# zrudnick/bramble

Hardware: AMD Instinct MI355X
Metric: projected alignments/sec vs GENCODE-scale annotation (higher is better)
Workload: dtype u32; 1 GPU; device-resident (inputs already in HBM, packed rows left in HBM): 10M paired-end 2x100 short reads (name-collated, unstranded) vs GENCODE-shaped synthetic annotation (250836 transcripts, 1684128 transcript-exon rows, 25 refs); BASELINE.json configs[1]; group_lanes=8, seed=0xb4a3b1e

## Files before the change

bramble_amd/csrc/direct_kernels.inc:

```

#define WAVE_SYNC()                                                \
  do {                                                             \
    __builtin_amdgcn_fence(__ATOMIC_RELEASE, "workgroup");         \
    __builtin_amdgcn_wave_barrier();                               \
    __builtin_amdgcn_fence(__ATOMIC_ACQUIRE, "workgroup");         \
  } while (0)

__global__ void __launch_bounds__(256) k_name_seed(DirectArgs D) {
  const int64_t g = (int64_t)blockIdx.x * blockDim.x + threadIdx.x;
  if (g >= D.n_groups) return;
  const uint32_t a0 = D.group_off[g];
  const uint32_t no = D.name_off[a0];
  Mt64Lazy gen;
  gen.seed(hash_bytes(D.names + no, D.name_off[a0 + 1] - no));
  D.rnd0[g] = gen();
}
__device__ __forceinline__ uint32_t pick_from(uint64_t z0, const uint8_t *name, uint64_t len, uint32_t n) {
  uint64_t hi, lo;
  mul64wide(z0, (uint64_t)n, hi, lo);
  if (lo < (uint64_t)n) {
    const uint64_t thr = (0 - (uint64_t)n) % (uint64_t)n;
    if (lo < thr) return primary_pick(name, len, n);
  }
  return (uint32_t)hi;
// ... 164 lines not shown
  __shared__ uint16_t sh_mops[EM ? 256 : 1];
  const int lane = threadIdx.x;
  if (EM) {
    for (int t = lane; t < 256; t += 64) sh_mops[t] = (uint16_t)((merge_action(t >> 4, t & 15u) << 8) | merge_ops(t >> 4, t & 15u));
    WAVE_SYNC();
  }
  const DevIndex &ix = A.ix;
  const DevCfg &cfg = A.cfg;
  const uint32_t n_work = *D.n_big;
  for (uint32_t w = blockIdx.x; w < n_work; w += gridDim.x) {
    if (D.side_used[1]) {
      if (EM) return;
      unsigned long long need = 0;
      for (uint64_t v = (uint64_t)w + (uint64_t)lane * gridDim.x; v < n_work; v += 64ull * gridDim.x) need += side_need(D.n_matches[D.big_list[v]]);
#pragma unroll
      for (int d = 32; d >= 1; d >>= 1) need += __shfl_down(need, d, 64);
      if (lane == 0 && need) atomicAdd(D.side_used, need);
      return;
    }
    const uint32_t a = D.big_list[w];
    const uint32_t nm = D.n_matches[a];
    if (EM && D.n_kept[a] == 0) continue;
    const uint4 hd = A.head[a], hd2 = A.head2[a], rg = A.ranges[a];
    const uint32_t n_seg = hd.z, rid = hd.w >> 2;
    if (n_seg == 0 || nm == 0) continue;
    const uint2 q0 = make_uint2(hd.x, hd.y);
    const int st0 = (n_seg == 1) ? ST_ONLY : ST_FIRST;
    const uint32_t sb[2] = {ix.slab_off[2 * rid], ix.slab_off[2 * rid + 1]}, se[2] = {ix.slab_off[2 * rid + 1], ix.slab_off[2 * rid + 2]};
    const uint32_t n0 = rg.y - rg.x, n_items = n0 + (rg.w - rg.z);
    unsigned long long off = 0;
    uint4 E = make_uint4(0, 0, 0, 0);
    if (!EM) {
      const unsigned long long need = side_need(nm);
      if (lane == 0) off = atomicAdd(D.side_used, need);
      off = ((unsigned long long)__shfl((uint32_t)(off >> 32), 0) << 32) | __shfl((uint32_t)off, 0);
      if (off + need > D.side_cap) { if (lane == 0) D.side_used[1] = 1; continue; }
      if (lane == 0) D.fm[a] = make_uint2((uint32_t)off, (uint32_t)(off >> 32));
    } else {
      const uint2 f = D.fm[a];
      off = (unsigned long long)f.x | ((unsigned long long)f.y << 32);
      { const uint2 gd = D.gd[a], dp = D.dpos[a]; E = make_uint4(gd.x, gd.y, dp.x, dp.y); }
    }
    const uint32_t c0 = A.cigar_off[a];
    ReadCtx rd;
    rd.n_seg = n_seg; rd.seg = A.seg + (size_t)c0 + (size_t)a; rd.real = A.cigar + c0; rd.n_real = A.cigar_off[a + 1] - c0; rd.q12 = hd2;
    uint32_t seen = 0;
    for (uint32_t base = 0; base < n_items; base += 64) {
// ... 359 lines not shown
  }
  sh_v[wv][lane] = v;
#pragma unroll
  for (int c = 0; c < 2; c++) {
    const uint32_t mine = (nk && fast == (c == 0)) ? nk : 0u;
    const uint64_t have = __ballot(mine != 0u);
    if (!have) continue;
    uint32_t inc = mine;
#pragma unroll
    for (int d = 1; d < 64; d <<= 1) { const uint32_t up = __shfl_up(inc, d); if (lane >= d) inc += up; }
    const uint32_t total = __shfl(inc, 63), first = __shfl(pos, (int)__builtin_ctzll(have));
    __builtin_amdgcn_wave_barrier();
    sh_pre[wv][lane] = inc - mine;
    WAVE_SYNC();
    for (uint32_t e = lane; e < total; e += 64) {
      int l = 0;
#pragma unroll
      for (int st = 32; st; st >>= 1) if (sh_pre[wv][l + st] <= e) l += st;
      D.m_aln[first + e] = sh_v[wv][l];
    }
  }
}

template <int CLS>
__global__ void __launch_bounds__(256, CLS == 1 ? 8 : 6) k_emit_rows(ProjectArgs A, DirectArgs D, int64_t first, int64_t n_end) {
  __shared__ uint32_t sh_cig[CLS == 1 ? 1 : 256 * LDS_SLOT];
  __shared__ uint16_t sh_mops[CLS == 1 ? 1 : 256];
  if (CLS != 1) {
    sh_mops[threadIdx.x] = (uint16_t)((merge_action(threadIdx.x >> 4, threadIdx.x & 15u) << 8) | merge_ops(threadIdx.x >> 4, threadIdx.x & 15u));
    __syncthreads();
  }
  const int64_t e64 = first + (int64_t)blockIdx.x * blockDim.x + threadIdx.x;
  if (e64 >= n_end) return;
  const DevIndex &ix = A.ix;
  const DevCfg &cfg = A.cfg;
  typedef uint32_t ntl4 __attribute__((ext_vector_type(4)));
  typedef uint32_t ntl2 __attribute__((ext_vector_type(2)));
  const uint32_t a = __builtin_nontemporal_load(D.m_aln + e64);
  if (a == 0xffffffffu) return;
  const ntl4 hd_ = __builtin_nontemporal_load((const ntl4 *)(A.head + a)), rg_ = __builtin_nontemporal_load((const ntl4 *)(A.ranges + a));
  const ntl2 f_ = __builtin_nontemporal_load((const ntl2 *)(D.fm + a)), gd_ = __builtin_nontemporal_load((const ntl2 *)(D.gd + a)), dp_ = __builtin_nontemporal_load((const ntl2 *)(D.dpos + a));
  const uint4 hd = make_uint4(hd_.x, hd_.y, hd_.z, hd_.w), rg = make_uint4(rg_.x, rg_.y, rg_.z, rg_.w);
  const uint2 f = make_uint2(f_.x, f_.y), gd = make_uint2(gd_.x, gd_.y), dp = make_uint2(dp_.x, dp_.y);
  const uint4 E = make_uint4(gd.x, gd.y, dp.x, dp.y);
  const uint32_t is_fast = CLS == 1;
  uint4 hd2 = make_uint4(0, 0, 0, 0);
  uint32_t c0 = 0, c1 = 0;
  RealCig rc;
  if (CLS != 1) { hd2 = A.head2[a]; c0 = A.cigar_off[a]; c1 = A.cigar_off[a + 1]; }
  else if (hd.z == 2) hd2 = A.head2[a];
  const uint32_t n_seg = hd.z, rid = hd.w >> 2;
  const uint2 q0 = make_uint2(hd.x, hd.y);
  const int st0 = (n_seg == 1) ? ST_ONLY : ST_FIRST;
  const uint32_t n0 = rg.y - rg.x;
  if (CLS != 1) rc.fetch(A.cigar + c0, c1 - c0);
  const uint32_t k = (uint32_t)e64 - E.w;
  const uint64_t fmask = (uint64_t)f.x | ((uint64_t)f.y << 32);
  uint64_t mm = fmask;
  for (uint32_t j = 0; j < k; j++) mm &= mm - 1;
  const uint32_t item = (uint32_t)(__ffsll((long long)mm) - 1);
  const int s = item < n0 ? 0 : 1;
  const uint32_t row = s == 0 ? rg.x + item : rg.z + (item - n0);
  const uint4 r_a = ix.s_row[2 * (size_t)row], r_b = ix.s_row[2 * (size_t)row + 1];
  const uint32_t gs = r_a.x, gend = r_a.y;
  const uint4 pay = make_uint4(r_b.x, r_b.y, r_a.w, r_b.z);
  uint32_t c = 0;
  {
    for (uint64_t m2 = fmask; m2;) {
      uint32_t t8[8]; bool ok[8];
#pragma unroll
      for (int u = 0; u < 8; u++) {
        ok[u] = m2 != 0;
        const uint32_t b = ok[u] ? (uint32_t)(__ffsll((long long)m2) - 1) : item;
        m2 &= m2 - 1;
        t8[u] = ix.s_tid[b < n0 ? rg.x + b : rg.z + (b - n0)];
      }
#pragma unroll
      for (int u = 0; u < 8; u++) c += (ok[u] && t8[u] < pay.x) ? 1u : 0u;
    }
  }
  Hit h0;
  classify(s == 1, st0, q0.x, q0.y, gs, gend, pay.z, cfg, h0);
  if (is_fast) {
    const uint32_t os = q0.x > gs ? q0.x : gs, oe = q0.y < gend ? q0.y : gend;
    uint32_t ml = oe - os, pos = h0.pos, r_ins = h0.right_ins, junc_in = 0;
    bool r_exact = h0.right_ins == 0 && h0.right_gap == 0;
    if (n_seg == 2) {
      const uint2 q1 = make_uint2(hd2.x, hd2.y);
      const uint4 e1 = next_row(make_uint4(gs, gend, pay.z, 0), make_uint2(r_a.z, r_b.w), s == 1);
      Hit hh;
      classify(s == 1, ST_LAST, q1.x, q1.y, e1.x, e1.y, e1.z, cfg, hh);
      ml += (q1.y < e1.y ? q1.y : e1.y) - q1.x;
      pos = s == 0 ? h0.pos : hh.pos;
      r_ins = hh.right_ins; r_exact = hh.right_ins == 0 && hh.right_gap == 0;
      junc_in = 2;
    }
    uint32_t w0, w1 = 0, w2 = 0, n_out;
    if (h0.left_ins) { w0 = CIG_GEN(h0.left_ins, OP_S); w1 = CIG_GEN(ml, OP_M); n_out = 2; if (r_ins) { w2 = CIG_GEN(r_ins, OP_S); n_out = 3; } }
    else { w0 = CIG_GEN(ml, OP_M); n_out = 1; if (r_ins) { w1 = CIG_GEN(r_ins, OP_S); n_out = 2; } }
    const uint32_t junc = junc_in + ((h0.left_ins == 0 && h0.left_gap == 0) ? 1u : 0u) + (r_exact ? 1u : 0u);
    uint64_t cref = (uint64_t)w0 | ((uint64_t)w1 << 32);
    if (n_out == 3) {
      cref = D.cig_base[a] + (uint64_t)c * (n_seg == 2 ? 3u + 2u * 10u : 1u + 2u * 6u);
      uint32_t *slot = A.cig_arena + cref;
      slot[0] = w0; slot[1] = w1; slot[2] = w2;
    }
    write_row(D, E, a, c, pay.x, pos, n_out, s == 1, cref, junc, ml);
    return;
  }
  if (CLS == 1) return;
  ReadCtx rd;
  rd.n_seg = n_seg; rd.seg = A.seg + (size_t)c0 + (size_t)a; rd.real = A.cigar + c0; rd.n_real = c1 - c0; rd.q12 = hd2;
  const uint4 *Ex = ix.tx_ex + pay.w;
  const uint32_t i0 = pay.y & 0x7fffffffu;
  CandOut p1;
  bool plain = false;
  const uint32_t sb = ix.slab_off[2 * rid + s], se = ix.slab_off[2 * rid + s + 1];
  if (n_seg == 1) { p1.alive = true; p1.fwpos = h0.pos; p1.rcpos = h0.pos; p1.n_seg = 1; p1.n_gex = 1; p1.i_lastm = i0; p1.last_right_ins = h0.right_ins; p1.last_right_gap = h0.right_gap; }
  else if (!cfg.long_reads && !cfg.ignore_small_exons) {
    plain = true;
    p1.alive = true; p1.fwpos = h0.pos; p1.rcpos = h0.pos; p1.n_seg = n_seg; p1.n_gex = n_seg; p1.i_lastm = i0;
    p1.last_right_ins = 0; p1.last_right_gap = 0;
  }
  else p1 = walk_pass1(ix, cfg, rd, Ex, s == 1, sb, se, i0, make_uint4(gs, gend, pay.z, 0), make_uint2(r_a.z, r_b.w), q0, h0);
  const uint32_t ideal_cap = 4u * n_seg + 2u;
  const uint32_t cap = rd.n_real + 2u * ideal_cap;
// ... 57 lines not shown
```

bramble_amd/csrc/kernels.h:

```cpp
#pragma once
#include <hip/hip_runtime.h>
#include <stdint.h>

#include "device_types.h"
#include "ksw_types.h"

namespace br {

enum {
  TOT_MATCHES = 0,
  TOT_ARENA = 1,
  TOT_SIMPLE = 2,
  TOT_ROWS = 3,
  TOT_RAW = 4,
  TOT_RESCUE_PROB = 5,
  TOT_RESCUE_SEQ = 6,
  TOT_WIDE_CIGAR = 7,
  TOT_SMALL_CNT = 8,
  TOT_PARSE_CIGAR = 12,
  TOT_PARSE_NAMES = 13,
  TOT_PARSE_GROUPS = 14,
  TOT_PARSE_SEQ = 15,
  TOT_BAM_LONG = 16,
  TOT_BAM_BYTES = 17,
// ... 355 lines not shown
};
struct SoaArgs {
  int64_t n;
  const uint64_t *cigar_off64, *name_off64, *seq_off64;
  uint32_t *cigar_off, *name_off, *seq_off;
  const uint8_t *names;
  const uint32_t *cigar;
  uint32_t *isnew;
  uint32_t *maxima;
};
void launch_soa_fields(hipStream_t st, const SoaArgs &S);
void launch_rec_fields(hipStream_t st, const ParseArgs &P);
void launch_group_off(hipStream_t st, const ParseArgs &P);
void launch_rec_copy(hipStream_t st, const ParseArgs &P);
void launch_mates(hipStream_t st, const ParseArgs &P);
void launch_seq_src(hipStream_t st, const ParseArgs &P);
void launch_seq_ascii(hipStream_t st, const ParseArgs &P);
void launch_bam_size(hipStream_t st, const BamArgs &B);
void launch_bam_encode(hipStream_t st, const BamArgs &B, int lanes);

struct SegExtra {
  const uint32_t *group_off; uint32_t *aln_group; int64_t n_groups;
  uint64_t *zero_a; int n_zero_a; uint64_t *zero_b; int n_zero_b;
};
void launch_segment(hipStream_t st, int64_t n_aln, const int32_t *ref_id, const int32_t *ref_start,
                    const uint16_t *flags, const int8_t *xs, const int8_t *ts, const uint32_t *cigar_off,
                    const uint32_t *cigar, const DevCfg &cfg, uint32_t n_refs, uint2 *seg, AlnMeta *meta,
                    uint4 *head, uint4 *head2, uint32_t *fast_flag, const SegExtra *extra = nullptr);
void launch_project(hipStream_t st, const ProjectArgs &A, bool emit, int group_lanes, int n_blocks);
void launch_count(hipStream_t st, const CountArgs &C, int group_lanes, int n_blocks, int part);
void launch_project_fa(hipStream_t st, const ProjectArgs &A, const FaArgs &F, int mode, int n_blocks);
void launch_fa_fill(hipStream_t st, const ProjectArgs &A, const FaArgs &F, int64_t n_prob);
void launch_ksw(hipStream_t st, const KswArgs &K, int n_blocks);
void launch_ksw_bin(hipStream_t st, const KswFastArgs &A);
void launch_ksw_dp(hipStream_t st, const KswFastArgs &A, int bin);
void launch_ksw_trace(hipStream_t st, const KswFastArgs &A, int bin);
uint32_t ksw_dp_resident_groups(int bin, int n_cu);
size_t ksw_prob_bytes();
size_t ksw_res_bytes();
void launch_expand(hipStream_t st, const ProjectArgs &A);
void launch_emit_dense(hipStream_t st, const ProjectArgs &A, int64_t n_matches, int64_t n_simple, int part);
void launch_emit_dense_fa(hipStream_t st, const ProjectArgs &A, const FaArgs &F, int64_t n_matches);
int64_t scan_tiles_for(int64_t n);
void launch_scan(hipStream_t st, const ScanArgs &S, int mode, void *out, bool out64, uint64_t *total_out);
void launch_group_ids(hipStream_t st, int64_t n_groups, const uint32_t *group_off, uint32_t *aln_group);
bool launch_scan3(hipStream_t st, ScanArgs S, uint32_t *match_off, uint64_t *cig_base, uint32_t *fast_pre,
                  uint64_t *total_out3, const ProjectArgs *expand = nullptr);
// ... 11 lines not shown
```

bramble_amd/csrc/pipeline.cpp:

```cpp
#include <algorithm>
#include <cstring>
#include <vector>

#include "ctx.h"

int ensure_side_stream(br_ctx *c) {
  if (c->side_stream) return BR_OK;
  HIPCHK(hipStreamCreateWithPriority(&c->side_stream, hipStreamNonBlocking, 0));
  for (auto &p : c->side_ev) for (auto &e : p) HIPCHK(hipEventCreateWithFlags(&e, hipEventDisableTiming));
  return BR_OK;
}

int run_ksw(br_ctx *c, hipStream_t st, const KswRun &R) {
  if (R.n_prob <= 0) return BR_OK;
  const uint64_t n_all = (uint64_t)R.n_prob;
  const uint64_t qmax = std::max<uint64_t>(R.qmax, 1), tmax = std::max<uint64_t>(R.tmax, 1);
  KswArgs K{};
  K.n_prob = R.n_prob; K.probs = R.probs; K.results = R.results; K.seq_arena = R.seq_arena; K.clip_ops = R.clip_ops;
  K.stats = R.stats;
  K.raw_out = R.raw_out; K.raw_n = R.raw_n; K.max_out = R.max_out; K.raw_cap = R.raw_cap;
  auto general = [&](uint64_t n_work, uint64_t q_hi, uint64_t t_hi, const uint32_t *list, const uint32_t *n_list) -> int {
    q_hi = std::max<uint64_t>(q_hi, 1); t_hi = std::max<uint64_t>(t_hi, 1);
    K.tmax = (uint32_t)t_hi;
    K.pmat_bytes = (size_t)(((q_hi + t_hi) * t_hi + 15) & ~15ull);
// ... 395 lines not shown
  RC(c->row_off.ensure((size_t)(n + 1) * 8));
  RC(ensure_side_stream(c));
  if (!c->side2_stream) HIPCHK(hipStreamCreateWithPriority(&c->side2_stream, hipStreamNonBlocking, 0));
  hipStream_t ax = c->side_stream, ax2 = c->side2_stream;
  uint64_t *d_tot = c->totals.as<uint64_t>();
  ReadBack *rb = c->rb;

  ProjectArgs A = count_args(c, dc, b);
  A.n_big = dz_nbig; A.walk_list = c->walk_list.as<uint32_t>(); A.n_walk = dz_nbig + 1;
  const bool have_names = b->names && b->name_off;
  DirectArgs D{};
  D.n_aln = n; D.n_groups = ng; D.group_off = b->group_off; D.aln_group = c->aln_group.as<uint32_t>(); D.mate_idx = b->mate_idx;
  D.n_matches = c->n_matches.as<uint32_t>(); D.mask = c->mask.as<uint64_t>(); D.ranges = c->ranges.as<uint4>();
  D.fast_flag = c->fast_flag.as<uint32_t>(); D.s_tid = ix->dev.s_tid; D.big_list = A.big_list; D.n_big = A.n_big;
  D.fm = c->d_fm.as<uint2>(); D.pm_list = (uint32_t *)(c->d_fm.as<uint2>() + n); D.pm_n = dz_nbig + 2; D.n_kept = c->d_nkept.as<uint32_t>(); D.n_rows = c->n_rows.as<uint32_t>(); D.pflag = c->pbit.as<uint8_t>();
  D.side = c->d_side.as<uint2>(); D.side_cap = c->d_side_cap; D.side_used = (unsigned long long *)(dz + GD_COUNTER_WORDS);
  D.cls_pos = c->d_clspos.as<uint32_t>(); D.cig_base = c->cig_base.as<uint64_t>(); D.row_off = c->row_off.as<uint64_t>();
  D.name_off = have_names ? b->name_off : nullptr; D.names = have_names ? b->names : nullptr; D.rnd0 = c->d_rnd.as<uint64_t>();
  D.gd = c->d_desc.as<uint2>(); D.dpos = c->d_desc.as<uint2>() + n; D.hi0 = c->d_hi0.as<uint32_t>(); D.counters = c->counters_d.as<uint64_t>(); D.tot = d_tot;

  SideWork seeds(c, st, ax2), pair_big(c, st, ax), group_desc(c, st, ax), big_emit(c, st, ax);
  HIPCHK(hipMemsetAsync(dz, 0, (GD_COUNTER_WORDS + 4) * 8, st));
  RC(pair_big.fork());
  RC(segment_stage(c, st, dc, b, pf));
  RC(pf.begin(BR_K_GROUP_IDS));
  launch_group_ids(st, ng, b->group_off, c->aln_group.as<uint32_t>());
  RC(pf.end());
  RC(count_pass(c, st, A, pf, true, true));
  if (c->rows_busy_set) { HIPCHK(hipStreamWaitEvent(st, c->rows_busy, 0)); }
  const int big_blocks = c->n_cu * 4;
  uint64_t kept = 0, arena = 0, n_simple = 0, n_rows = 0, n_raw = 0;
  bool expanded_ahead = false;
  if (have_names) {
    RC(seeds.fork());
    RC(pf.begin(BR_K_NAME_SEED, ax2));
    launch_name_seed(ax2, D);
    RC(pf.end());
    RC(seeds.done());
  }
  for (int attempt = 0;; attempt++) {
    if (attempt) {
      HIPCHK(hipMemsetAsync(dz, 0, (GD_COUNTER_WORDS + 2) * 8, st));
      HIPCHK(hipMemsetAsync(D.pm_n, 0, 4, st));
    }
    RC(pair_big.fork());
    RC(pf.begin(BR_K_PAIR_BIG, ax));
    launch_big_collect(ax, A, D, big_blocks);
// ... 365 lines not shown
  uint64_t n = (uint64_t)b->n_aln;
  c->counters[3] = h[3]; c->counters[4] = h[4]; c->counters[5] = h[5]; c->counters[7] = h[7];
  c->counters[0] = 24ull * n + 4ull * h[3];
  c->counters[1] = h[1];
  c->counters[2] = 4ull * n + 24ull * (uint64_t)nm + 4ull * h[7];
  return BR_OK;
}

extern "C" int br_ctx_direct_diag(br_ctx *c, uint64_t out[8], uint8_t *pflags) {
  if (!c || !out || !c->last_direct) return BR_ERR_INVALID_ARG;
  HIPCHK(hipSetDevice(c->ix->device));
  const DirectArgs &D = c->dD;
  uint64_t used = 0;
  uint32_t nb[3] = {0, 0, 0};
  HIPCHK(hipDeviceSynchronize());
  HIPCHK(hipMemcpy(&used, D.side_used, 8, hipMemcpyDeviceToHost));
  HIPCHK(hipMemcpy(nb, D.n_big, 12, hipMemcpyDeviceToHost));
  if (pflags && D.n_aln > 0) HIPCHK(hipMemcpy(pflags, D.pflag, (size_t)D.n_aln, hipMemcpyDeviceToHost));
  memset(out, 0, 8 * sizeof(uint64_t));
  out[0] = nb[0]; out[1] = (uint64_t)c->d_side_attempts; out[2] = used; out[3] = D.side_cap; out[4] = nb[2];
  if (D.n_aln > 0) {
    const size_t n = (size_t)D.n_aln;
    std::vector<uint32_t> ff(n), nk(n);
    std::vector<uint4> hd(n);
    std::vector<uint8_t> pf(n);
    HIPCHK(hipMemcpy(ff.data(), D.fast_flag, n * 4, hipMemcpyDeviceToHost));
    HIPCHK(hipMemcpy(nk.data(), D.n_kept, n * 4, hipMemcpyDeviceToHost));
    HIPCHK(hipMemcpy(hd.data(), c->head.p, n * sizeof(uint4), hipMemcpyDeviceToHost));
    HIPCHK(hipMemcpy(pf.data(), D.pflag, n, hipMemcpyDeviceToHost));
    uint64_t light = 0;
    for (size_t a = 0; a < n; a++)
      if ((ff[a] >> 31) && hd[a].z == 2 && !(pf[a] & PF_BIG)) light += nk[a];
    out[5] = light;
  }
  return BR_OK;
}

extern "C" int br_project_batch_device(br_ctx *c, const br_config *cfg, const br_device_batch *b, void *stream,
                                       br_device_rows *out) {
  if (!c || !cfg || !b || !out) return BR_ERR_INVALID_ARG;
  return run_device(c, cfg, b, (hipStream_t)stream, out);
}

extern "C" int br_device_rows_expand(br_ctx *c, void *stream, br_device_wide_rows *out) {
  if (!c || !out) return BR_ERR_INVALID_ARG;
  return expand_rows(c, (hipStream_t)stream, out);
}
```

bramble_amd/csrc/project_kernels.hip:

```cpp
#include <hip/hip_runtime.h>
#include <stdint.h>

#include <algorithm>

#include "device_types.h"
#include "kernels.h"
#include "primary_pick.h"

namespace br {

#define CIG_OP(c) ((c) & 0xfu)
#define CIG_LEN(c) ((c) >> 4)
#define CIG_GEN(l, o) (((l) << 4) | (o))

__global__ void __launch_bounds__(256) k_segment(int64_t n_aln, const int32_t *__restrict__ ref_id,
                                                 const int32_t *__restrict__ ref_start,
                                                 const uint16_t *__restrict__ flags,
                                                 const int8_t *__restrict__ xs, const int8_t *__restrict__ ts,
                                                 const uint32_t *__restrict__ cigar_off,
                                                 const uint32_t *__restrict__ cigar, DevCfg cfg,
                                                 uint32_t n_refs, uint2 *__restrict__ seg,
                                                 AlnMeta *__restrict__ meta, uint4 *__restrict__ head,
                                                 uint4 *__restrict__ head2, uint32_t *__restrict__ fast_flag, SegExtra X) {
  int64_t a = (int64_t)blockIdx.x * blockDim.x + threadIdx.x;
// ... 60 lines not shown
      bool cond = (cfg.rf && is_rev) || (cfg.fr && !is_rev);
      if (f & 0x1) {
        int order = (f & 0x40) ? 1 : ((f & 0x80) ? 2 : 0);
        strand = (order == 1) ? (cond ? '-' : '+') : (cond ? '+' : '-');
      } else {
        strand = cond ? '-' : '+';
      }
    }
    smode = (strand == '+') ? 1u : (strand == '-') ? 2u : 3u;
  }
  uint32_t lclip = 0, rclip = 0;
  if (cfg.long_reads) {
    if (n_cigar == 0) { n = 0; }
    else {
      uint32_t w0 = cg[0];
      if (CIG_OP(w0) == OP_H) { if (n_cigar > 1 && CIG_OP(cg[1]) == OP_S) lclip = CIG_LEN(cg[1]); }
      else if (CIG_OP(w0) == OP_S) lclip = CIG_LEN(w0);
      uint32_t wl = cg[n_cigar - 1];
      if (CIG_OP(wl) == OP_H) { if (n_cigar >= 2 && CIG_OP(cg[n_cigar - 2]) == OP_S) rclip = CIG_LEN(cg[n_cigar - 2]); }
      else if (CIG_OP(wl) == OP_S) rclip = CIG_LEN(wl);
    }
  }
  if (cfg.long_reads) { AlnMeta m; m.n_seg = n; m.smode = smode; m.n_left_clip = lclip; m.n_right_clip = rclip; meta[a] = m; }
  uint2 q0 = n ? e0 : make_uint2(0, 0);
  head[a] = make_uint4(q0.x, q0.y, n, n ? (((uint32_t)rid << 2) | smode) : 0u);
  if (n > 1) {
    const bool mnm = n == 2 && n_cigar == 3 && pre4 && CIG_OP(w4[0]) == OP_M && CIG_OP(w4[2]) == OP_M && !cfg.filter_by_similarity &&
                     !cfg.long_reads && !cfg.ignore_small_exons;
    const uint2 q2 = n > 2 ? e2 : make_uint2(mnm ? 1u : 0u, 0);
    head2[a] = make_uint4(e1.x, e1.y, q2.x, q2.y);
  }
  uint32_t fast = (n == 1 && n_cigar == 1 && CIG_OP(cg[0]) == OP_M && !cfg.filter_by_similarity && !cfg.long_reads) ? 1u : 0u;
  fast_flag[a] = (fast << 31) | ((n_cigar + 2u * (4u * n + 2u)) & 0x7fffffffu);
}

struct Hit { uint32_t pos, left_ins, right_ins, left_gap, right_gap; };

__device__ __forceinline__ bool classify(bool minus, int status, uint32_t qs, uint32_t qe, uint32_t s,
                                         uint32_t e, uint32_t pos_start, const DevCfg &c, Hit &h) {
  const bool junc_left = (status == ST_MIDDLE || status == ST_LAST);
  const bool junc_right = (status == ST_FIRST || status == ST_MIDDLE);
  const uint32_t lg = qs > s ? qs - s : 0u, li = s > qs ? s - qs : 0u;
  const uint32_t rg = e > qe ? e - qe : 0u, ri = qe > e ? qe - e : 0u;
  const uint32_t lim_li = junc_left ? c.max_junc_ins : c.max_clip;
  const uint32_t lim_ri = (junc_right || minus) ? c.max_junc_ins : c.max_clip;
  const uint32_t lim_lg = junc_left ? c.max_junc_gap : 0xffffffffu;
  const uint32_t lim_rg = junc_right ? c.max_junc_gap : 0xffffffffu;
  h.pos = pos_start + (minus ? rg : lg); h.left_ins = li; h.right_ins = ri; h.left_gap = lg; h.right_gap = rg;
  return (li <= lim_li) & (ri <= lim_ri) & (lg <= lim_lg) & (rg <= lim_rg);
}

struct IdealSink {
  uint32_t *buf; uint32_t n; uint32_t cur; bool has;
  __device__ __forceinline__ void init(uint32_t *b) { buf = b; n = 0; cur = 0; has = false; }
  __device__ __forceinline__ void add(uint32_t len, uint32_t op) {
// ... 463 lines not shown
  const Ix groups_total = (Ix)gridDim.x * per_block;
  const Ix gid = (Ix)blockIdx.x * per_block + threadIdx.x / G;
  const DevIndex &ix = proj_index(A);
  const DevCfg &cfg = proj_cfg<PRE>(A);
  const uint32_t n_slab_off = 2 * ix.n_refs + 1;
  const bool slab_in_lds = n_slab_off <= SLAB_LDS;
  if (slab_in_lds) {
    for (uint32_t i = threadIdx.x; i < n_slab_off; i += blockDim.x) {
      sh_slab[i] = ix.slab_off[i];
      if (!EMIT && i <= ix.n_refs) sh_bin[i] = ix.bin_off[i];
    }
    __syncthreads();
  }

  if constexpr (EMIT) { if (tot_over(A.tot, A.lim_m, A.lim_c)) return; }
  const Ix n_work = EMIT ? (Ix)*A.n_big : MODE == 2 ? (Ix)*A.n_walk : (Ix)A.n_aln;
  for (Ix w = gid; w < n_work; w += groups_total) {
    const Ix a = EMIT ? (Ix)A.big_list[w] : MODE == 2 ? (Ix)A.walk_list[w] : w;
    uint4 hd = A.head[a];
    uint4 hd2 = A.head2[a];
    uint32_t n_seg = hd.z;
    if (EMIT && n_seg == 0) continue;
    uint2 q0 = make_uint2(hd.x, hd.y);
    uint32_t smode = hd.w & 3u, rid = hd.w >> 2;
    int st0 = (n_seg == 1) ? ST_ONLY : ST_FIRST;
    uint32_t sb[2], se[2];
    if (slab_in_lds) { sb[0] = sh_slab[2 * rid]; se[0] = sh_slab[2 * rid + 1]; se[1] = sh_slab[2 * rid + 2]; }
    else { sb[0] = ix.slab_off[2 * rid]; se[0] = ix.slab_off[2 * rid + 1]; se[1] = ix.slab_off[2 * rid + 2]; }
    sb[1] = se[0];

    uint32_t lo[2] = {0, 0}, hi[2] = {0, 0};
    if constexpr (EMIT) {
      if (A.n_matches[a] == 0) continue;
      uint4 rg = A.ranges[a];
      lo[0] = rg.x; hi[0] = rg.y; lo[1] = rg.z; hi[1] = rg.w;
    } else {
      uint32_t tw[4];
      const uint32_t bo = slab_in_lds ? sh_bin[rid] : ix.bin_off[rid];
      const uint32_t nb = (slab_in_lds ? sh_bin[rid + 1] : ix.bin_off[rid + 1]) - bo - 1;
      uint32_t bh = q0.y >> ix.bin_shift, bl = q0.x >> ix.bin_shift;
      bh = bh < nb - 1 ? bh : nb - 1; bl = bl < nb - 1 ? bl : nb - 1;
      {
        const uint4 tl = ix.t_bin[bo + bl], th = ix.t_bin[bo + bh + 1];
        tw[0] = tl.x; tw[1] = th.y; tw[2] = tl.z; tw[3] = th.w;
      }
#pragma unroll
      for (int s = 0; s < 2; s++) {
// ... 181 lines not shown
          A.m_x[mi] = make_uint2((uint32_t)acc.junc_hits, (uint32_t)acc.ref_consumed);
          if (SIMF) {
            unsigned long long sb64 = (unsigned long long)__double_as_longlong(score);
            A.m_b[mi] = make_uint4((uint32_t)acc.clip_score, 0u, (uint32_t)sb64, (uint32_t)(sb64 >> 32));
          }
          A.m_cigoff[mi] = cig_ref;
        }
      }
      if (EMIT && !have_mask && sweep == 0) __threadfence_block();
    }
    if (MODE == 1 && ((__ballot(defer) >> gbase) & gmask) != 0) {
      if (gl == 0) {
        uint32_t k = atomicAdd(&sh_wn, 1u);
        if (k < WALK_LDS) sh_wl[MODE == 1 ? k : 0] = (uint32_t)a;
        else { uint32_t k2 = atomicAdd(A.n_walk, 1u); A.walk_list[k2] = (uint32_t)a; }
      }
      continue;
    }
    bool light = false;
    if constexpr (MODE == 1 && CNT && PRE == 1)
      light = n_seg == 2 && hd2.z != 0 && n_items <= 64 && ((__ballot(inexact != 0u) >> gbase) & gmask) == 0;
    if (!EMIT && gl == 0) {
      A.n_matches[a] = total; A.mask[a] = mask_all;
      if constexpr (MODE == 1 && CNT && PRE == 1) { if (light && A.light_flag) A.light_flag[a] = (1u << 31) | (3u + 2u * (4u * 2u + 2u)); }
      if (n_items > 64 && total) {
        const uint32_t k = atomicAdd(&sh_bn, 1u);
        if (k < BIG_LDS) sh_bl[EMIT ? 0 : k] = (uint32_t)a;
        else { const uint32_t k2 = atomicAdd(A.n_big, 1u); A.big_list[k2] = (uint32_t)a; }
      }
    }
  }
  if (!EMIT) {
    __syncthreads();
    const uint32_t n_loc = sh_bn < BIG_LDS ? sh_bn : BIG_LDS;
    if (threadIdx.x == 0) sh_bbase = n_loc ? atomicAdd(A.n_big, n_loc) : 0u;
    __syncthreads();
    for (uint32_t i = threadIdx.x; i < n_loc; i += blockDim.x) A.big_list[sh_bbase + i] = sh_bl[EMIT ? 0 : i];
  }
  if (MODE == 1) {
    __syncthreads();
    const uint32_t n_loc = sh_wn < WALK_LDS ? sh_wn : WALK_LDS;
    if (threadIdx.x == 0) sh_wbase = n_loc ? atomicAdd(A.n_walk, n_loc) : 0u;
    __syncthreads();
    for (uint32_t i = threadIdx.x; i < n_loc; i += blockDim.x) A.walk_list[sh_wbase + i] = sh_wl[MODE == 1 ? i : 0];
  }
}

// ... 49 lines not shown
    __syncthreads();
  }
  if (A.tot) {
    if (tot_over(A.tot, A.lim_m, A.lim_c)) return;
    n_matches = CLS == 1 ? (int64_t)A.tot[TOT_SIMPLE] : (int64_t)A.tot[TOT_MATCHES];
    first = CLS == 2 ? (int64_t)A.tot[TOT_SIMPLE] : 0;
    if ((uint64_t)(n_matches - first) > A.cover) return;
  }
  int64_t mi64 = first + (int64_t)blockIdx.x * blockDim.x + threadIdx.x;
  if (mi64 >= n_matches) return;
  const DevIndex &ix = A.ix;
  const DevCfg &cfg = A.cfg;
  uint32_t a = A.m_aln[mi64];
  if (a == 0xffffffffu) return;
  uint4 hd = A.head[a];
  uint4 hd2 = A.head2[a];
  uint4 rg = A.ranges[a];
  uint64_t mask = A.mask[a];
  const uint32_t part_fast = CLS == 1 ? 1u : CLS == 2 ? 0u : (A.fast_flag[a] >> 31);
  const uint32_t is_fast = FA ? 0u : part_fast;
  uint32_t moff = A.match_off[a];
  uint64_t cbase = A.cig_base[a];
  uint32_t c0 = A.cigar_off[a], c1 = A.cigar_off[a + 1];
  uint32_t n_seg = hd.z, rid = hd.w >> 2;
  uint2 q0 = make_uint2(hd.x, hd.y);
  int st0 = (n_seg == 1) ? ST_ONLY : ST_FIRST;
  uint32_t n0 = rg.y - rg.x;
  RealCig rc;
  if (CLS != 1) rc.fetch(A.cigar + c0, c1 - c0);
  const uint32_t fpre = A.fast_pre[a];
  uint32_t k = (uint32_t)mi64 - (part_fast ? fpre : A.fast_pre[A.n_aln] + (moff - fpre));
  uint64_t mm = mask;
  for (uint32_t j = 0; j < k; j++) mm &= mm - 1;
  uint32_t item = (uint32_t)(__ffsll((long long)mm) - 1);
  int s = item < n0 ? 0 : 1;
  uint32_t row = s == 0 ? rg.x + item : rg.z + (item - n0);
  const uint4 r_a = ix.s_row[2 * (size_t)row], r_b = ix.s_row[2 * (size_t)row + 1];
  uint32_t gs = r_a.x, gend = r_a.y;
  uint4 pay = make_uint4(r_b.x, r_b.y, r_a.w, r_b.z);
  uint32_t rank = 0;
  for (uint64_t m2 = mask; m2;) {
    uint32_t t8[8]; bool ok[8];
#pragma unroll
    for (int u = 0; u < 8; u++) {
      ok[u] = m2 != 0;
      uint32_t b = ok[u] ? (uint32_t)(__ffsll((long long)m2) - 1) : item;
      m2 &= m2 - 1;
// ... 1029 lines not shown
```

bramble_amd/csrc/rescue_kernels.inc:

```

__device__ __forceinline__ uint8_t base_code(uint8_t c) {
  switch (c) { case 'A': case 'a': return 0; case 'C': case 'c': return 1; case 'G': case 'g': return 2;
               case 'T': case 't': return 3; default: return 4; }
}

struct FaCand {
  bool alive;
  bool wantL, wantR;
  uint32_t qlenL, tlenL, qlenR, tlenR;
};

__device__ __forceinline__ uint32_t target_len(const uint4 *E, uint32_t i_from, bool leftwards, uint32_t qlen) {
  uint32_t acc = 0;
  if (leftwards) { for (uint32_t i = i_from; acc < qlen; i--) { acc += E[i].y - E[i].x; if (i == 0) break; } }
  else { for (uint32_t i = i_from; acc < qlen && E[i].x != 0xffffffffu; i++) acc += E[i].y - E[i].x; }
  uint32_t cap = qlen + 40u;
  return acc < cap ? acc : cap;
}

template <int MODE, int G>
__global__ void __launch_bounds__(256) k_project_fa(ProjectArgs A, FaArgs F) {
  const int gl = threadIdx.x & (G - 1);
  const int gbase = (threadIdx.x & 63) & ~(G - 1);
  const uint64_t gmask = (G == 64) ? ~0ull : ((1ull << G) - 1ull);
  auto gballot = [&](bool x) -> uint64_t { return (__ballot(x) >> gbase) & gmask; };
  const int64_t groups_total = (int64_t)gridDim.x * (blockDim.x / G);
  const int64_t gid = (int64_t)blockIdx.x * (blockDim.x / G) + threadIdx.x / G;
  const DevIndex &ix = A.ix;
  const DevCfg &cfg = A.cfg;

  for (int64_t a = gid; a < A.n_aln; a += groups_total) {
    uint4 hd = A.head[a];
    uint32_t n_seg = hd.z;
    if (n_seg == 0) {
      if (gl == 0) {
        if (MODE == 0) { F.n_prob[a] = 0; F.seq_bytes[a] = 0; A.ranges[a] = make_uint4(0, 0, 0, 0); }
        if (MODE == 2) { A.n_matches[a] = 0; F.ideal_cap[a] = 0; }
      }
      continue;
    }
    if (MODE == 3 && A.n_matches[a] == 0) continue;
    if (MODE == 3) { const uint4 rg3 = A.ranges[a]; if ((rg3.y - rg3.x) + (rg3.w - rg3.z) <= 64u) continue; }
    uint2 q0 = make_uint2(hd.x, hd.y);
    uint32_t smode = hd.w & 3u, rid = hd.w >> 2;
    int st0 = (n_seg == 1) ? ST_ONLY : ST_FIRST;
    uint32_t sb[2], se[2];
    sb[0] = ix.slab_off[2 * rid]; se[0] = ix.slab_off[2 * rid + 1]; se[1] = ix.slab_off[2 * rid + 2]; sb[1] = se[0];
    uint32_t lo[2] = {0, 0}, hi[2] = {0, 0};
    if (MODE != 0) { uint4 rg = A.ranges[a]; lo[0] = rg.x; hi[0] = rg.y; lo[1] = rg.z; hi[1] = rg.w; }
    else {
#pragma unroll
      for (int s = 0; s < 2; s++) {
        lo[s] = hi[s] = sb[s];
        if (!((smode >> s) & 1u) || sb[s] == se[s]) continue;
        uint32_t bo = ix.bin_off[rid], nb = ix.bin_off[rid + 1] - bo - 1;
        uint32_t bh = q0.y >> ix.bin_shift, bl = q0.x >> ix.bin_shift;
        bh = bh < nb - 1 ? bh : nb - 1; bl = bl < nb - 1 ? bl : nb - 1;
        const uint4 th0 = ix.t_bin[bo + bh], th1 = ix.t_bin[bo + bh + 1], tl0 = ix.t_bin[bo + bl], tl1 = ix.t_bin[bo + bl + 1];
        uint32_t ha = s ? th0.w : th0.y, hb = s ? th1.w : th1.y, la = s ? tl0.z : tl0.x, lb = s ? tl1.z : tl1.x;
        uint32_t ch = 0, cl = 0;
        for (uint32_t r0 = ha; r0 < hb; r0 += G) { uint32_t r = r0 + gl; ch += (uint32_t)__popcll(gballot(r < hb && ix.s_start[r] < q0.y)); }
        for (uint32_t r0 = la; r0 < lb; r0 += G) { uint32_t r = r0 + gl; cl += (uint32_t)__popcll(gballot(r < lb && ix.s_pmax[r] <= q0.x)); }
        hi[s] = ha + ch; lo[s] = la + cl < hi[s] ? la + cl : hi[s];
      }
      if (gl == 0) A.ranges[a] = make_uint4(lo[0], hi[0], lo[1], hi[1]);
    }
    uint32_t n0 = hi[0] - lo[0], n1 = hi[1] - lo[1], n_items = n0 + n1;
// ... 181 lines not shown
```

bramble_amd/lib.py:

```python
import ctypes as C
import os

import numpy as np

_HERE = os.path.dirname(os.path.abspath(__file__))
LIB_PATH = os.path.join(_HERE, "libbramble_amd.so")
_P = C.POINTER

K_SEGMENT, K_COUNT, K_EMIT, K_PAIR_COUNT, K_PAIR_EMIT, K_GATHER, K_SCAN, K_EMIT_AUX, K_KSW, K_BAM, K_PARSE, K_CODEC, K_EMIT_SIMPLE, K_PRIMARY, K_CIGAR_POOL, K_COUNT_WALK, K_EXPAND, K_GROUP_IDS, K_P1, K_P1_WALK, K_EMIT_WL, K_NAME_SEED, K_PAIR_MASK, K_PAIR_BIG, K_GROUP_DESC, K_EXPAND_ROWS, K_EMIT_ROWS_SIMPLE, K_EMIT_ROWS, K_BIG_EMIT, K_SAM_FORMAT, K_NUM = range(31)
KERNEL_NAMES = ["k_segment", "k_project<G,false,false,1>", "k_emit_dense<false,2>", "k_pair<false>", "k_pair<true>",
                "k_rows", "k_scan_*", "k_project<64,true>", "k_ksw", "k_bam_scan+k_bam_size+k_bam_encode",
                "k_rec_fields+k_group_off+k_rec_copy+k_mates+k_seq_*", "k_deflate_*+k_bgzf_compact",
                "k_emit_dense<false,1>", "k_primary", "(unused)", "k_project<G,false,false,2>", "k_expand", "k_group_ids",
                "(unused)", "(unused)", "(unused)", "k_name_seed", "k_pair_mask", "k_big<0>+k_pair_big", "k_group_desc",
                "k_expand_rows", "k_emit_rows<1>", "k_emit_rows<2>", "k_big<1>", "k_samfmt_*"]


class BrambleError(RuntimeError):
    pass


class BrExon(C.Structure):
    _fields_ = [("start", C.c_uint32), ("end", C.c_uint32)]

# ... 520 lines not shown
        db.max_n_cigar = dev_batch["max_n_cigar"]
        if dev_batch.get("seqs") is not None:
            db.seq_off = dev_batch["seq_off"].data_ptr()
            db.seqs = dev_batch["seqs"].data_ptr()
            db.seq_src = dev_batch["seq_src"].data_ptr()
            db.max_soft_clip = dev_batch["max_soft_clip"]
        if dev_batch.get("names") is not None:
            db.name_off = dev_batch["name_off"].data_ptr()
            db.names = dev_batch["names"].data_ptr()
        return db

    def collect_counters(self, dev_batch, stream=0):
        db = self._device_batch_struct(dev_batch)
        check(lib().br_ctx_collect_counters(self.h, C.byref(db), C.c_void_p(stream)), "br_ctx_collect_counters")
        out = (C.c_uint64 * 8)()
        check(lib().br_ctx_last_counters(self.h, out), "br_ctx_last_counters")
        keys = ("B_in", "B_idx", "B_out", "n_cigar", "read_exons", "overlap_hits", "matches", "out_cigar_words")
        return dict(zip(keys, [int(v) for v in out]))

    def direct_diag(self, n_aln=None):
        out = (C.c_uint64 * 8)()
        pf = np.zeros(n_aln, dtype=np.uint8) if n_aln is not None else None
        check(lib().br_ctx_direct_diag(self.h, out, pf.ctypes.data if pf is not None and n_aln else None), "br_ctx_direct_diag")
        d = dict(zip(("n_big", "side_attempts", "side_used", "side_cap", "pm_n", "light"), [int(v) for v in out[:6]]))
        if pf is not None:
            d["pflags"] = pf
        return d

    def project_bam_device(self, cfg, blob, rec_off, rec_len, ref_map, stream=0):
        recs = BrDeviceRecords()
        recs.blob = blob.data_ptr()
        recs.rec_off = rec_off.data_ptr()
        recs.n_aln = rec_len.numel()
        recs.rec_len = rec_len.data_ptr()
        rm = np.ascontiguousarray(ref_map, dtype=np.int32)
        rows, out = BrDeviceRows(), BrDeviceBam()
        check(lib().br_project_bam_device(self.h, C.byref(cfg), C.byref(recs), rm.ctypes.data, len(rm), C.c_void_p(stream),
                                          C.byref(rows), C.byref(out)), "br_project_bam_device")
        return rows, out

    def bgzf_deflate_device(self, src, stream=0):
        import torch
        from .device import _DevArray
        out, n = C.c_void_p(), C.c_uint64()
        check(lib().br_bgzf_deflate_device(self.h, C.c_void_p(src.data_ptr()), src.numel(), C.c_void_p(stream), C.byref(out),
                                           C.byref(n)), "br_bgzf_deflate_device")
        if n.value == 0:
# ... 483 lines not shown
```

Measured before the change: 3.116 billion alignments/s.

## Route soft-clipped single-segment and spliced reads through fast emit path

Single-segment reads whose CIGAR is S/M, M/S or S/M/S are now flagged as fast. Their clip lengths are packed into head2 and a new bit 31 of the head word, so k_emit_rows<1> handles them instead of the general CIGAR-walking path. Two-segment spliced reads with a single leading or trailing soft clip are also marked light, with the clip lengths carried in head2. This adds bit packing to the header (the rid field is masked to 29 bits) and extra head2 loads and stores. A compile-time knob is added for the occupancy of the class-2 emit kernel.

```diff
diff --git a/bramble_amd/csrc/direct_kernels.inc b/bramble_amd/csrc/direct_kernels.inc
--- a/bramble_amd/csrc/direct_kernels.inc
+++ b/bramble_amd/csrc/direct_kernels.inc
@@ -210,7 +210,7 @@
     const uint32_t nm = D.n_matches[a];
     if (EM && D.n_kept[a] == 0) continue;
     const uint4 hd = A.head[a], hd2 = A.head2[a], rg = A.ranges[a];
-    const uint32_t n_seg = hd.z, rid = hd.w >> 2;
+    const uint32_t n_seg = hd.z, rid = HEAD_RID(hd.w);
     if (n_seg == 0 || nm == 0) continue;
     const uint2 q0 = make_uint2(hd.x, hd.y);
     const int st0 = (n_seg == 1) ? ST_ONLY : ST_FIRST;
@@ -616,8 +616,11 @@
   }
 }
 
+#ifndef BR_EMIT2_WAVES
+#define BR_EMIT2_WAVES 6
+#endif
 template <int CLS>
-__global__ void __launch_bounds__(256, CLS == 1 ? 8 : 6) k_emit_rows(ProjectArgs A, DirectArgs D, int64_t first, int64_t n_end) {
+__global__ void __launch_bounds__(256, CLS == 1 ? 8 : BR_EMIT2_WAVES) k_emit_rows(ProjectArgs A, DirectArgs D, int64_t first, int64_t n_end) {
   __shared__ uint32_t sh_cig[CLS == 1 ? 1 : 256 * LDS_SLOT];
   __shared__ uint16_t sh_mops[CLS == 1 ? 1 : 256];
   if (CLS != 1) {
@@ -642,8 +645,8 @@
   uint32_t c0 = 0, c1 = 0;
   RealCig rc;
   if (CLS != 1) { hd2 = A.head2[a]; c0 = A.cigar_off[a]; c1 = A.cigar_off[a + 1]; }
-  else if (hd.z == 2) hd2 = A.head2[a];
-  const uint32_t n_seg = hd.z, rid = hd.w >> 2;
+  else if (hd.z == 2 || HEAD_CLIP1(hd.w)) hd2 = A.head2[a];
+  const uint32_t n_seg = hd.z, rid = HEAD_RID(hd.w);
   const uint2 q0 = make_uint2(hd.x, hd.y);
   const int st0 = (n_seg == 1) ? ST_ONLY : ST_FIRST;
   const uint32_t n0 = rg.y - rg.x;
@@ -689,13 +692,16 @@
       r_ins = hh.right_ins; r_exact = hh.right_ins == 0 && hh.right_gap == 0;
       junc_in = 2;
     }
+    const uint32_t cl = hd2.w & 0xffffu, cr = hd2.w >> 16;
+    const uint32_t l_s = cl + h0.left_ins, r_s = cr + r_ins;
     uint32_t w0, w1 = 0, w2 = 0, n_out;
-    if (h0.left_ins) { w0 = CIG_GEN(h0.left_ins, OP_S); w1 = CIG_GEN(ml, OP_M); n_out = 2; if (r_ins) { w2 = CIG_GEN(r_ins, OP_S); n_out = 3; } }
-    else { w0 = CIG_GEN(ml, OP_M); n_out = 1; if (r_ins) { w1 = CIG_GEN(r_ins, OP_S); n_out = 2; } }
+    if (l_s) { w0 = CIG_GEN(l_s, OP_S); w1 = CIG_GEN(ml, OP_M); n_out = 2; if (r_s) { w2 = CIG_GEN(r_s, OP_S); n_out = 3; } }
+    else { w0 = CIG_GEN(ml, OP_M); n_out = 1; if (r_s) { w1 = CIG_GEN(r_s, OP_S); n_out = 2; } }
     const uint32_t junc = junc_in + ((h0.left_ins == 0 && h0.left_gap == 0) ? 1u : 0u) + (r_exact ? 1u : 0u);
     uint64_t cref = (uint64_t)w0 | ((uint64_t)w1 << 32);
     if (n_out == 3) {
-      cref = D.cig_base[a] + (uint64_t)c * (n_seg == 2 ? 3u + 2u * 10u : 1u + 2u * 6u);
+      const uint32_t n_cigar = 2u * n_seg - 1u + (cl ? 1u : 0u) + (cr ? 1u : 0u);
+      cref = D.cig_base[a] + (uint64_t)c * (n_cigar + 2u * (4u * n_seg + 2u));
       uint32_t *slot = A.cig_arena + cref;
       slot[0] = w0; slot[1] = w1; slot[2] = w2;
     }
diff --git a/bramble_amd/csrc/kernels.h b/bramble_amd/csrc/kernels.h
--- a/bramble_amd/csrc/kernels.h
+++ b/bramble_amd/csrc/kernels.h
@@ -401,7 +401,10 @@
 struct SegExtra {
   const uint32_t *group_off; uint32_t *aln_group; int64_t n_groups;
   uint64_t *zero_a; int n_zero_a; uint64_t *zero_b; int n_zero_b;
-};
+  uint32_t clip_simple;
+};
+#define HEAD_RID(w) (((w) >> 2) & 0x1fffffffu)
+#define HEAD_CLIP1(w) ((w) >> 31)
 void launch_segment(hipStream_t st, int64_t n_aln, const int32_t *ref_id, const int32_t *ref_start,
                     const uint16_t *flags, const int8_t *xs, const int8_t *ts, const uint32_t *cigar_off,
                     const uint32_t *cigar, const DevCfg &cfg, uint32_t n_refs, uint2 *seg, AlnMeta *meta,
diff --git a/bramble_amd/csrc/pipeline.cpp b/bramble_amd/csrc/pipeline.cpp
--- a/bramble_amd/csrc/pipeline.cpp
+++ b/bramble_amd/csrc/pipeline.cpp
@@ -441,7 +441,9 @@
   SideWork seeds(c, st, ax2), pair_big(c, st, ax), group_desc(c, st, ax), big_emit(c, st, ax);
   HIPCHK(hipMemsetAsync(dz, 0, (GD_COUNTER_WORDS + 4) * 8, st));
   RC(pair_big.fork());
-  RC(segment_stage(c, st, dc, b, pf));
+  SegExtra X{};
+  X.clip_simple = 1;
+  RC(segment_stage(c, st, dc, b, pf, &X));
   RC(pf.begin(BR_K_GROUP_IDS));
   launch_group_ids(st, ng, b->group_off, c->aln_group.as<uint32_t>());
   RC(pf.end());
@@ -853,15 +855,20 @@
   if (D.n_aln > 0) {
     const size_t n = (size_t)D.n_aln;
     std::vector<uint32_t> ff(n), nk(n);
-    std::vector<uint4> hd(n);
+    std::vector<uint4> hd(n), hd2(n);
     std::vector<uint8_t> pf(n);
     HIPCHK(hipMemcpy(ff.data(), D.fast_flag, n * 4, hipMemcpyDeviceToHost));
     HIPCHK(hipMemcpy(nk.data(), D.n_kept, n * 4, hipMemcpyDeviceToHost));
     HIPCHK(hipMemcpy(hd.data(), c->head.p, n * sizeof(uint4), hipMemcpyDeviceToHost));
+    HIPCHK(hipMemcpy(hd2.data(), c->head2.p, n * sizeof(uint4), hipMemcpyDeviceToHost));
     HIPCHK(hipMemcpy(pf.data(), D.pflag, n, hipMemcpyDeviceToHost));
-    uint64_t light = 0;
-    for (size_t a = 0; a < n; a++)
-      if ((ff[a] >> 31) && hd[a].z == 2 && !(pf[a] & PF_BIG)) light += nk[a];
+    uint64_t light = 0, clipped = 0;
+    for (size_t a = 0; a < n; a++) {
+      if (!(ff[a] >> 31) || (pf[a] & PF_BIG)) continue;
+      if (hd[a].z == 2) light += nk[a];
+      if ((hd[a].z == 2 || HEAD_CLIP1(hd[a].w)) && hd2[a].w != 0) clipped += nk[a];
+    }
+    out[6] = clipped;
     out[5] = light;
   }
   return BR_OK;
diff --git a/bramble_amd/csrc/project_kernels.hip b/bramble_amd/csrc/project_kernels.hip
--- a/bramble_amd/csrc/project_kernels.hip
+++ b/bramble_amd/csrc/project_kernels.hip
@@ -106,15 +106,36 @@
     }
   }
   if (cfg.long_reads) { AlnMeta m; m.n_seg = n; m.smode = smode; m.n_left_clip = lclip; m.n_right_clip = rclip; meta[a] = m; }
+  const bool short_plain = pre4 && !cfg.filter_by_similarity && !cfg.long_reads;
+  const uint32_t o0 = CIG_OP(w4[0]), o1 = CIG_OP(w4[1]), o2 = CIG_OP(w4[2]), o3 = CIG_OP(w4[3]);
+  if (n > 1) {
+    uint32_t mark = 0, clips = 0;
+    if (n == 2 && short_plain && !cfg.ignore_small_exons) {
+      uint32_t len = 0;
+      if (n_cigar == 3 && o0 == OP_M && o2 == OP_M) mark = 3;
+      else if (n_cigar == 4 && o0 == OP_S && o1 == OP_M && o3 == OP_M) { mark = 4; len = CIG_LEN(w4[0]); clips = len; }
+      else if (n_cigar == 4 && o0 == OP_M && o2 == OP_M && o3 == OP_S) { mark = 4; len = CIG_LEN(w4[3]); clips = len << 16; }
+      if (mark == 4 && (len == 0 || len > 0xffffu)) mark = 0;
+    }
+    const uint2 q2 = n > 2 ? e2 : make_uint2(mark, mark ? clips : 0u);
+    head2[a] = make_uint4(e1.x, e1.y, q2.x, q2.y);
+  }
+  uint32_t clip1 = 0;
+  if (X.clip_simple && n == 1 && short_plain && (uint32_t)rid < (1u << 29)) {
+    const uint32_t l0 = CIG_LEN(w4[0]), l1 = CIG_LEN(w4[1]), l2 = CIG_LEN(w4[2]);
+    uint32_t cl = 0, cr = 0;
+    bool ok = false;
+    if (n_cigar == 2 && o0 == OP_S && o1 == OP_M) { ok = true; cl = l0; }
+    else if (n_cigar == 2 && o0 == OP_M && o1 == OP_S) { ok = true; cr = l1; }
+    else if (n_cigar == 3 && o0 == OP_S && o1 == OP_M && o2 == OP_S) { ok = l0 != 0 && l2 != 0; cl = l0; cr = l2; }
+    if (ok && (cl | cr) != 0 && cl <= 0xffffu && cr <= 0xffffu) {
+      clip1 = 1;
+      head2[a] = make_uint4(0, 0, 0, cl | (cr << 16));
+    }
+  }
   uint2 q0 = n ? e0 : make_uint2(0, 0);
-  head[a] = make_uint4(q0.x, q0.y, n, n ? (((uint32_t)rid << 2) | smode) : 0u);
-  if (n > 1) {
-    const bool mnm = n == 2 && n_cigar == 3 && pre4 && CIG_OP(w4[0]) == OP_M && CIG_OP(w4[2]) == OP_M && !cfg.filter_by_similarity &&
-                     !cfg.long_reads && !cfg.ignore_small_exons;
-    const uint2 q2 = n > 2 ? e2 : make_uint2(mnm ? 1u : 0u, 0);
-    head2[a] = make_uint4(e1.x, e1.y, q2.x, q2.y);
-  }
-  uint32_t fast = (n == 1 && n_cigar == 1 && CIG_OP(cg[0]) == OP_M && !cfg.filter_by_similarity && !cfg.long_reads) ? 1u : 0u;
+  head[a] = make_uint4(q0.x, q0.y, n, n ? ((clip1 << 31) | ((uint32_t)rid << 2) | smode) : 0u);
+  uint32_t fast = ((n == 1 && n_cigar == 1 && CIG_OP(cg[0]) == OP_M && !cfg.filter_by_similarity && !cfg.long_reads) || clip1) ? 1u : 0u;
   fast_flag[a] = (fast << 31) | ((n_cigar + 2u * (4u * n + 2u)) & 0x7fffffffu);
 }
 
@@ -624,7 +645,7 @@
     uint32_t n_seg = hd.z;
     if (EMIT && n_seg == 0) continue;
     uint2 q0 = make_uint2(hd.x, hd.y);
-    uint32_t smode = hd.w & 3u, rid = hd.w >> 2;
+    uint32_t smode = hd.w & 3u, rid = HEAD_RID(hd.w);
     int st0 = (n_seg == 1) ? ST_ONLY : ST_FIRST;
     uint32_t sb[2], se[2];
     if (slab_in_lds) { sb[0] = sh_slab[2 * rid]; se[0] = sh_slab[2 * rid + 1]; se[1] = sh_slab[2 * rid + 2]; }
@@ -852,7 +873,7 @@
       light = n_seg == 2 && hd2.z != 0 && n_items <= 64 && ((__ballot(inexact != 0u) >> gbase) & gmask) == 0;
     if (!EMIT && gl == 0) {
       A.n_matches[a] = total; A.mask[a] = mask_all;
-      if constexpr (MODE == 1 && CNT && PRE == 1) { if (light && A.light_flag) A.light_flag[a] = (1u << 31) | (3u + 2u * (4u * 2u + 2u)); }
+      if constexpr (MODE == 1 && CNT && PRE == 1) { if (light && A.light_flag) A.light_flag[a] = (1u << 31) | (hd2.z + 2u * (4u * 2u + 2u)); }
       if (n_items > 64 && total) {
         const uint32_t k = atomicAdd(&sh_bn, 1u);
         if (k < BIG_LDS) sh_bl[EMIT ? 0 : k] = (uint32_t)a;
@@ -948,7 +969,7 @@
   uint32_t moff = A.match_off[a];
   uint64_t cbase = A.cig_base[a];
   uint32_t c0 = A.cigar_off[a], c1 = A.cigar_off[a + 1];
-  uint32_t n_seg = hd.z, rid = hd.w >> 2;
+  uint32_t n_seg = hd.z, rid = HEAD_RID(hd.w);
   uint2 q0 = make_uint2(hd.x, hd.y);
   int st0 = (n_seg == 1) ? ST_ONLY : ST_FIRST;
   uint32_t n0 = rg.y - rg.x;
diff --git a/bramble_amd/csrc/rescue_kernels.inc b/bramble_amd/csrc/rescue_kernels.inc
--- a/bramble_amd/csrc/rescue_kernels.inc
+++ b/bramble_amd/csrc/rescue_kernels.inc
@@ -42,7 +42,7 @@
     if (MODE == 3 && A.n_matches[a] == 0) continue;
     if (MODE == 3) { const uint4 rg3 = A.ranges[a]; if ((rg3.y - rg3.x) + (rg3.w - rg3.z) <= 64u) continue; }
     uint2 q0 = make_uint2(hd.x, hd.y);
-    uint32_t smode = hd.w & 3u, rid = hd.w >> 2;
+    uint32_t smode = hd.w & 3u, rid = HEAD_RID(hd.w);
     int st0 = (n_seg == 1) ? ST_ONLY : ST_FIRST;
     uint32_t sb[2], se[2];
     sb[0] = ix.slab_off[2 * rid]; se[0] = ix.slab_off[2 * rid + 1]; se[1] = ix.slab_off[2 * rid + 2]; sb[1] = se[0];
diff --git a/bramble_amd/lib.py b/bramble_amd/lib.py
--- a/bramble_amd/lib.py
+++ b/bramble_amd/lib.py
@@ -566,7 +566,7 @@
         out = (C.c_uint64 * 8)()
         pf = np.zeros(n_aln, dtype=np.uint8) if n_aln is not None else None
         check(lib().br_ctx_direct_diag(self.h, out, pf.ctypes.data if pf is not None and n_aln else None), "br_ctx_direct_diag")
-        d = dict(zip(("n_big", "side_attempts", "side_used", "side_cap", "pm_n", "light"), [int(v) for v in out[:6]]))
+        d = dict(zip(("n_big", "side_attempts", "side_used", "side_cap", "pm_n", "light", "clipped"), [int(v) for v in out[:7]]))
         if pf is not None:
             d["pflags"] = pf
         return d
```

Result: no change. 3.105 billion alignments/s (-0.4%).
